# acmater/prograph

Hardware: AMD Instinct MI355X
Metric: sequence-pairs/s (higher is better)
Workload: dtype u8; 1 GPU; cfg3: N=200000 L=64 Hamming, kNN k=16; N=200000, L=64, rows_per_gpu=200000, alphabet=5-bit tokens 1..20, parallelism=rowblock1, engine=mfma

## Files before the change

### prograph_amd/csrc/pg_api.hip

```cpp
#include "pg_common.h"
#include "pg_mm.h"
#include "pg_plan.h"
#include "../../include/prograph_hip.h"

#include <dlfcn.h>
#include <math.h>
#include <rccl/rccl.h>
#include <stdio.h>
#include <stdlib.h>
#include <string.h>
#include <atomic>
#include <mutex>

static thread_local char g_err[256] = "";

void pg_set_error(const char *msg) { snprintf(g_err, sizeof(g_err), "%s", msg); }

extern char **environ;
static PgKnobs read_knobs() { return pg_knobs_read(environ); }

#define PG_MAX_DEVICES 64
static int cu_count() {
  static std::atomic<int> cus[PG_MAX_DEVICES];
  int dev = 0;
  if (hipGetDevice(&dev) != hipSuccess) return 0;
  const bool cached = dev >= 0 && dev < PG_MAX_DEVICES;
  if (cached && cus[dev].load(std::memory_order_relaxed) > 0) return cus[dev].load(std::memory_order_relaxed);
  hipDeviceProp_t prop;
  if (hipGetDeviceProperties(&prop, dev) != hipSuccess) return 0;
  if (cached) cus[dev].store(prop.multiProcessorCount, std::memory_order_relaxed);
  return prop.multiProcessorCount;
}

extern "C" {

int pg_version(void) { return PG_ABI_VERSION; }
const char *pg_last_error(void) { return g_err; }

int pg_device_info(int *cus, int *wave, char *arch, int arch_len) {
  int dev = 0;
  hipDeviceProp_t prop;
  hipError_t e = hipGetDevice(&dev);
  if (e != hipSuccess) return pg_launched((int)e, "hipGetDevice");
  e = hipGetDeviceProperties(&prop, dev);
  if (e != hipSuccess) return pg_launched((int)e, "hipGetDeviceProperties");
  if (cus) *cus = prop.multiProcessorCount;
  if (wave) *wave = prop.warpSize;
  if (arch && arch_len > 0) snprintf(arch, (size_t)arch_len, "%s", prop.gcnArchName);
  return 0;
}

int64_t pg_npad(int64_t n) { return n <= 0 ? 256 : ((n + 255) / 256) * 256; }
int pg_ngroups(int l) { return plan_ngroups(l); }
int pg_nchunks(int l, int bits) { return plan_nchunks(l, bits); }
int64_t pg_planes_bytes(int64_t n, int l, int bits) { return ((int64_t)pg_nchunks(l, bits) * 16 + PG_AUX_BYTES) * pg_npad(n); }
int64_t pg_workspace_bytes(int64_t nrows) { return workspace_bytes(nrows, cu_count(), read_knobs()); }

}

struct SymPlanArgs {
  long long nb, nst, slots;
  int piece, pmin;
  int4 *plan;
  u32 *pieceStart;
  uint4 *zero;
  long long zero4;
  unsigned grid;
};
static __device__ __forceinline__ void sym_plan_workgroup(unsigned vb, unsigned vgrid, const SymPlanArgs &a) {
  __shared__ u32 waveTotal[16];
  const int t = threadIdx.x, lane = t & 63, wv = t >> 6;
  if (vb > 0) {
    for (long long i = (long long)(vb - 1) * 1024 + t; i < a.zero4; i += (long long)(vgrid - 1) * 1024) a.zero[i] = make_uint4(0u, 0u, 0u, 0u);
    return;
  }
  const long long nb = a.nb, per = (nb + 1023) / 1024, b0 = t * per, b1 = b0 + per < nb ? b0 + per : nb;
  const bool few = per <= 4;
  u32 np4 = 0u, mine = 0;
  if (few) {
#pragma unroll 1
    for (int j = 0; b0 + j < b1; ++j) {
      const u32 np = (u32)sym_block_pieces(b0 + j, a.nst, a.slots, a.piece, a.pmin);
      np4 |= np << (8 * j);
      mine += np;
    }
  } else {
#pragma clang loop vectorize(disable) interleave(disable) unroll(disable)
    for (long long b = b0; b < b1; ++b) mine += (u32)sym_block_pieces(b, a.nst, a.slots, a.piece, a.pmin);
  }
  u32 incl = mine;
#pragma unroll
  for (int o = 1; o < 64; o <<= 1) {
    const u32 x = (u32)__shfl_up((int)incl, o);
    incl += lane >= o ? x : 0u;
  }
  if (lane == 63) waveTotal[wv] = incl;
  __syncthreads();
  u32 front = 0, total = 0;
#pragma unroll
  for (int i = 0; i < 16; ++i) {
    const u32 x = waveTotal[i];
    front += i < wv ? x : 0u;
    total += x;
  }
  u32 at = front + incl - mine;
  auto entries = [&](long long b, int np) {
    a.pieceStart[b] = at;
#pragma unroll 1
    for (int q = 0; q < np; ++q, ++at) {
      int f, e;
      sym_piece_range(b, a.nst, np, q, &f, &e);
      a.plan[at] = make_int4((int)b, f, e, q);
    }
  };
  if (few) {
#pragma unroll 1
    for (int j = 0; b0 + j < b1; ++j) entries(b0 + j, (int)((np4 >> (8 * j)) & 0xFFu));
  } else {
#pragma clang loop vectorize(disable) interleave(disable) unroll(disable)
    for (long long b = b0; b < b1; ++b) entries(b, sym_block_pieces(b, a.nst, a.slots, a.piece, a.pmin));
  }
  if (t == 1023) a.pieceStart[nb] = total;
}
__global__ __launch_bounds__(1024) void pg_knn_sym_plan_kernel(SymPlanArgs a) { sym_plan_workgroup(blockIdx.x, gridDim.x, a); }
extern "C" {
int64_t pg_knn_sym_plan(int64_t n, int64_t slots, int piece, int piece_min, int32_t *out, int64_t max_passes) {
  if (n <= 0 || slots <= 0) return pg_fail(PG_E_BADARG, "pg_knn_sym_plan: bad argument");
  return sym_plan_host(n, slots, piece, piece_min > 0 ? piece_min : (int)read_knobs().symPieceMin.v, out, max_passes);
}
int64_t pg_knn_sym_plan_device(int64_t n, int64_t slots, int piece, int piece_min, int32_t *plan_out, uint32_t *piece_start_out,
                               int64_t max_passes, void *stream) {
  if (n <= 0 || n > PG_MAX_N_KNN || slots <= 0 || !plan_out || !piece_start_out) return pg_fail(PG_E_BADARG, "pg_knn_sym_plan_device: bad argument");
  const int pmin = piece_min > 0 ? piece_min : (int)read_knobs().symPieceMin.v;
  const int64_t passes = sym_plan_host(n, slots, piece, pmin, nullptr, 0);
  if (passes > max_passes) return pg_fail(PG_E_BADARG, "pg_knn_sym_plan_device: the plan has more passes than max_passes");
  SymPlanArgs a = {(n + 63) / 64, (n + PG_MM_ST - 1) / PG_MM_ST, slots, piece, pmin, (int4 *)plan_out, piece_start_out, nullptr, 0, 1u};
  pg_knn_sym_plan_kernel<<<dim3(1), dim3(1024), 0, (hipStream_t)stream>>>(a);
  if (int rc = pg_launched("pg_knn_sym_plan_kernel")) return rc;
  return passes;
}
}

#define PG_PACK_SEQS 64
#define PG_PACK_LD 68

__host__ __device__ __forceinline__ unsigned long long pg_transpose8(unsigned long long x) {
  unsigned long long t;
  t = (x ^ (x >> 7)) & 0x00AA00AA00AA00AAull;  x = x ^ t ^ (t << 7);
  t = (x ^ (x >> 14)) & 0x0000CCCC0000CCCCull; x = x ^ t ^ (t << 14);
  t = (x ^ (x >> 28)) & 0x00000000F0F0F0F0ull; x = x ^ t ^ (t << 28);
  return x;
}

template <typename T, int B>
__global__ __launch_bounds__(256) void pg_pack_kernel(const T *__restrict__ src, long long n, int l, long long ld,
                                                      const long long *__restrict__ rows, u32 *__restrict__ planes,
                                                      long long npad, int ng, int nq, u32 *flags,
                                                      const unsigned char *__restrict__ lut = nullptr,
                                                      unsigned char *__restrict__ tokOut = nullptr) {
  constexpr int E = (int)sizeof(T), PER = 16 / E;
  __shared__ __attribute__((aligned(16))) u32 words[PG_PACK_SEQS * PG_PACK_LD];
  const long long s0 = (long long)blockIdx.x * PG_PACK_SEQS;
  const int tid = threadIdx.x;
  const bool vec = !lut && ((unsigned long long)src & 15ull) == 0 && ((ld * E) & 15ll) == 0;
  for (int item = tid; item < PG_PACK_SEQS * ng; item += 256) {
    const int sl = item / ng, g = item - sl * ng;
    const long long s = s0 + sl;
    unsigned long long x[4] = {0, 0, 0, 0}, high = 0;
    if (s < n) {
      const T *row = src + (rows ? rows[s] : s) * ld;
      if (vec && g * 32 + 32 <= l) {
        const uint4 *r16 = reinterpret_cast<const uint4 *>(row + g * 32);
#pragma unroll
        for (int c = 0; c < 32 / PER; ++c) {
          const uint4 v = r16[c];
          T e[PER];
          __builtin_memcpy(e, &v, 16);
#pragma unroll
          for (int i = 0; i < PER; ++i) {
            const int j = c * PER + i;
            const unsigned long long t = (unsigned long long)(long long)e[i];
            high |= t;
            x[j >> 3] |= (t & 0xFFull) << (8 * (j & 7));
          }
        }
      } else {
#pragma unroll
        for (int j = 0; j < 32; ++j) {
          const int pos = g * 32 + j;
          if (pos < l) {
            long long v = (long long)row[pos];
            if (lut) {
              v = lut[(unsigned char)v];
              if (tokOut) tokOut[s * (long long)l + pos] = (unsigned char)v;
            }
            high |= (unsigned long long)v;
            x[j >> 3] |= ((unsigned long long)v & 0xFFull) << (8 * (j & 7));
          }
        }
      }
    }
    if (high >> B) atomicOr(flags, 1u);
#pragma unroll
    for (int i = 0; i < 4; ++i) x[i] = pg_transpose8(x[i]);
#pragma unroll
    for (int p = 0; p < B; ++p) {
      const u32 w = (u32)((x[0] >> (8 * p)) & 0xFFull) | (u32)((x[1] >> (8 * p)) & 0xFFull) << 8 |
                    (u32)((x[2] >> (8 * p)) & 0xFFull) << 16 | (u32)((x[3] >> (8 * p)) & 0xFFull) << 24;
      words[sl * PG_PACK_LD + p * ng + g] = w;
    }
  }
  __syncthreads();
  const int nw = ng * B;
  for (int item = tid; item < PG_PACK_SEQS * nq; item += 256) {
    const int q = item / PG_PACK_SEQS, sl = item % PG_PACK_SEQS;
    uint4 v = *reinterpret_cast<const uint4 *>(&words[sl * PG_PACK_LD + 4 * q]);
    if (4 * q + 1 >= nw) v.y = 0;
    if (4 * q + 2 >= nw) v.z = 0;
    if (4 * q + 3 >= nw) v.w = 0;
    reinterpret_cast<uint4 *>(planes)[(long long)q * npad + s0 + sl] = v;
  }
  const int sl = tid & 63;
  const long long s = s0 + sl;
  if (tid < 64) {
    u32 sigw[2] = {0, 0};
    for (int g = 0; g < ng; ++g) sigw[g & 1] ^= words[sl * PG_PACK_LD + g];
    const unsigned long long sig = pg_sig54(sigw[0], sigw[1]);
    const u32 lo = (u32)sig, hi = (u32)(sig >> 32) | (s < n ? 0xFFC00000u : 0u);
    uint4 *e = reinterpret_cast<uint4 *>(planes + (long long)nq * npad * 4) + (s >> 5) * 64 + (s & 31);
    e[0] = make_uint4(pg_nib8(lo) << 1, pg_nib8(lo >> 8) << 1, pg_nib8(lo >> 16) << 1, pg_nib8(lo >> 24) << 1);
    e[32] = make_uint4(pg_nib8(hi) << 1, pg_nib8(hi >> 8) << 1, pg_nib8(hi >> 16) << 1, pg_nib8(hi >> 24) << 1);
  } else if (tid < 128) {
    u32 fold[8] = {0, 0, 0, 0, 0, 0, 0, 0};
#pragma unroll
    for (int p = 0; p < B; ++p)
      for (int g = 0; g < ng; ++g) fold[p] ^= words[sl * PG_PACK_LD + p * ng + g];
    uint4 *f = reinterpret_cast<uint4 *>(planes + (long long)nq * npad * 4) + npad * 2;
    f[s] = make_uint4(fold[0], fold[1], fold[2], fold[3]);
    f[npad + s] = make_uint4(fold[4], fold[5], fold[6], fold[7]);
  }
}

#define PG_SCAN_TILE 2048

template <typename T>
__device__ __forceinline__ long long scan_val(const T *in, long long i, long long n) {
  return i < n ? (long long)(in[i] != 0 ? (sizeof(T) == 1 ? 1 : in[i]) : 0) : 0;
}

__device__ __forceinline__ long long wave_incl_scan(long long v, int lane) {
#pragma unroll
  for (int o = 1; o < 64; o <<= 1) {
    long long t = __shfl_up(v, o);
    if (lane >= o) v += t;
  }
  return v;
}

__device__ __forceinline__ long long block_excl_scan(long long v, long long &total) {
  __shared__ long long wsum[4];
  const int lane = threadIdx.x & 63, wv = threadIdx.x >> 6;
  const long long inc = wave_incl_scan(v, lane);
  if (lane == 63) wsum[wv] = inc;
  __syncthreads();
  long long base = 0;
  for (int w = 0; w < wv; ++w) base += wsum[w];
  total = wsum[0] + wsum[1] + wsum[2] + wsum[3];
  __syncthreads();
  return base + inc - v;
}

template <typename T>
__global__ __launch_bounds__(256) void pg_scan_partials(const T *__restrict__ in, long long n, long long *partials) {
  const long long b0 = (long long)blockIdx.x * PG_SCAN_TILE;
  long long s = 0;
#pragma unroll
  for (int j = 0; j < 8; ++j) s += scan_val(in, b0 + threadIdx.x * 8 + j, n);
  long long total;
  block_excl_scan(s, total);
  if (threadIdx.x == 0) partials[blockIdx.x] = total;
}

__global__ __launch_bounds__(256) void pg_scan_single(long long *partials, long long nb) {
  long long carry = 0;
  for (long long c0 = 0; c0 < nb; c0 += 256) {
    const long long i = c0 + threadIdx.x;
    const long long v = i < nb ? partials[i] : 0;
    long long total;
    const long long ex = block_excl_scan(v, total);
    if (i < nb) partials[i] = carry + ex;
    carry += total;
  }
  if (threadIdx.x == 0) partials[nb] = carry;
}

template <typename T, int MODE>
__global__ __launch_bounds__(256) void pg_scan_apply(const T *__restrict__ in, long long n, const long long *partials,
                                                     long long nb, long long *out, long long *count) {
  const long long b0 = (long long)blockIdx.x * PG_SCAN_TILE;
  long long v[8], s = 0;
#pragma unroll
  for (int j = 0; j < 8; ++j) { v[j] = scan_val(in, b0 + threadIdx.x * 8 + j, n); s += v[j]; }
  long long total;
  long long ex = block_excl_scan(s, total) + partials[blockIdx.x];
#pragma unroll
  for (int j = 0; j < 8; ++j) {
    const long long i = b0 + threadIdx.x * 8 + j;
    if (i < n) {
      if (MODE == 0) out[i] = ex;
      else if (v[j]) out[ex] = i;
    }
    ex += v[j];
  }
  if (blockIdx.x == 0 && threadIdx.x == 0) {
    if (MODE == 0) out[n] = partials[nb];
    if (count) *count = partials[nb];
  }
}

template <int B>
__global__ __launch_bounds__(256) void pg_index_kernel(const u32 *__restrict__ planes, long long n, long long npad, int ng,
                                                       long long ref, const u32 *__restrict__ want, int posMode,
                                                       const u32 *__restrict__ posMask, const u32 *__restrict__ notMask,
                                                       unsigned char *distOut, u64 *hist, unsigned char *flags) {
  __shared__ u32 lh[256];
  lh[threadIdx.x] = 0;
  __syncthreads();
  const long long s = (long long)blockIdx.x * 256 + threadIdx.x;
  if (s < n) {
    u32 d = 0, anyP = 0, anyNot = 0;
    bool allP = true;
    for (int g = 0; g < ng; ++g) {
      u32 t = 0;
#pragma unroll
      for (int p = 0; p < B; ++p) {
        const int w = p * ng + g;
        const long long base = (long long)(w >> 2) * npad;
        t |= planes[(base + s) * 4 + (w & 3)] ^ planes[(base + ref) * 4 + (w & 3)];
      }
      d += __builtin_popcount(t);
      if (posMode) {
        const u32 pm = posMask[g], nm = notMask[g];
        anyP |= t & pm;
        allP = allP && ((t & pm) == pm);
        anyNot |= t & nm;
      }
    }
    if (distOut) distOut[s] = (unsigned char)d;
    if (hist) atomicAdd(&lh[d & 255u], 1u);
    if (flags) {
      bool ok = want ? ((want[(d >> 5) & 7u] >> (d & 31u)) & 1u) != 0 : true;
      if (posMode == 1) ok = ok && (anyP != 0) && (anyNot == 0);
      if (posMode == 2) ok = ok && allP && (anyNot == 0);
      flags[s] = ok ? 1 : 0;
    }
  }
  __syncthreads();
  if (hist && lh[threadIdx.x]) atomicAdd((unsigned long long *)&hist[threadIdx.x], (unsigned long long)lh[threadIdx.x]);
}

__device__ __forceinline__ double wave_sum(double v) {
#pragma unroll
  for (int o = 32; o > 0; o >>= 1) v += __shfl_down(v, o);
  return v;
}

__global__ __launch_bounds__(256) void pg_csr_row_stats_kernel(const long long *__restrict__ indptr,
                                                               const int *__restrict__ indices,
                                                               const unsigned char *__restrict__ w8,
                                                               const float *__restrict__ wf, long long nrows,
                                                               long long row0, const double *__restrict__ f, double *deg,
                                                               double *sf, double *swf, double *selfw, double *colsum) {
  const int lane = threadIdx.x & 63;
  const long long row = (long long)blockIdx.x * 4 + (threadIdx.x >> 6);
  if (row >= nrows) return;
  const long long a = indptr[row], b = indptr[row + 1];
  double d = 0, s1 = 0, s2 = 0, sw = 0;
  for (long long e = a + lane; e < b; e += 64) {
    const double w = w8 ? (double)w8[e] : (wf ? (double)wf[e] : 1.0);
    const int col = indices[e];
    if (col < 0) continue;
    const double fj = f ? f[col] : 0.0;
    d += w; s1 += fj; s2 += w * fj;
    if (col == row0 + row) sw += w;
    if (colsum) atomicAdd(&colsum[col], w);
  }
  d = wave_sum(d); s1 = wave_sum(s1); s2 = wave_sum(s2); sw = wave_sum(sw);
  if (lane == 0) {
    if (deg) deg[row] = d;
    if (sf) sf[row] = s1;
    if (swf) swf[row] = s2;
    if (selfw) selfw[row] = sw;
  }
}

static int check_l(int l, int bits = 8, bool exact = false) {
  if (l <= 0) return pg_fail(PG_E_BADARG, "sequence length must be positive");
  const int maxg = bits == 5 ? PG_MAX_L_5BIT / 32 + 1 : PG_MAX_L / 32;
  if ((l + 31) / 32 > maxg || (exact && l > (bits == 5 ? PG_MAX_L_5BIT : PG_MAX_L)))
    return pg_fail(PG_E_TOOLONG, "sequence length exceeds the native limit (128 tokens, 255 with 5 bit planes)");
  return 0;
}
static int check_bits(int b) {
  if (b != PG_BITS_5 && b != PG_BITS_8) return pg_fail(PG_E_BADARG, "bits must be 5 or 8");
  return 0;
}

static void eps_interval(int cmp, double eps, u32 *lo, u32 *span, long long dmin = 1) {
  const long long INF = 1000000;
  long long l = dmin, h = INF;
  switch (cmp) {
    case PG_CMP_LE: h = (long long)floor(eps); break;
    case PG_CMP_LT: h = (long long)ceil(eps) - 1; break;
    case PG_CMP_EQ:
      if (floor(eps) == eps) { l = (long long)eps; h = (long long)eps; } else { l = 1; h = 0; }
      break;
    case PG_CMP_GE: l = (long long)ceil(eps); break;
    case PG_CMP_GT: l = (long long)floor(eps) + 1; break;
  }
  if (l < dmin) l = dmin;
  if (h > INF) h = INF;
  if (h < l) { *lo = 0xFFFFFF00u; *span = 0; return; }
  *lo = (u32)l;
  *span = (u32)(h - l);
}

__global__ __launch_bounds__(1024) void pg_decide_kernel(const u32 *counts, int nsample, int wavesPerRow, u32 need, long long ncols,
                                                          int force, u32 *gate, u32 *line, int lineWords, SymPlanArgs ride) {
  if (blockIdx.x > 0) { sym_plan_workgroup(blockIdx.x - 1u, gridDim.x - 1u, ride); return; }
  __shared__ u32 sClustered[16];
  __shared__ unsigned long long sEps[16], sNear[16];
  const int tid = threadIdx.x, s = tid >> 4, sub = tid & 15;
  if (tid < lineWords) line[tid] = 0u;
  u32 nearS = 0, epsS = 0;
  if (s < nsample)
    for (int w = sub; w < wavesPerRow; w += 16) {
      nearS += counts[2 * (s * wavesPerRow + w)];
      epsS += counts[2 * (s * wavesPerRow + w) + 1];
    }
  for (int o = 8; o > 0; o >>= 1) {
// ... 1131 lines not shown
```

### prograph_amd/csrc/pg_plan.h

```cpp
#pragma once
#include "../../include/prograph_hip.h"

#include <math.h>
#include <stdint.h>
#include <stdlib.h>
#include <string.h>
#include <mutex>

#ifdef __HIPCC__
#define PG_HD __host__ __device__
#else
#define PG_HD
#endif

#ifndef PG_MODE_KNN_SHORT
enum { PG_MODE_EPS = 0, PG_MODE_KNN = 1, PG_MODE_EPS_SYM = 2 };
#define PG_MODE_KNN_SHORT 3
#define PG_MODE_KNN_SHORT2 4
#define PG_WG_WAVES 4
#define PG_RB 32
#define PG_RB_KNN 28
#define PG_MM_KL 20
#define PG_MM_RB 32
#define PG_MM_ST 128
#define PG_MM_DENSE_L1 56
#define PG_MM_DENSE_L2 48
#define PG_MM_DIRECT_RUN 8
#define PG_SYM_MAX_PIECES 16
#define PG_SYM_MAX_CAPL 256
#endif
static_assert(PG_MODE_KNN == 1 && PG_MODE_KNN_SHORT == 3 && PG_MODE_KNN_SHORT2 == 4 && PG_WG_WAVES == 4 && PG_RB == 32 &&
                  PG_RB_KNN == 28 && PG_MM_KL == 20 && PG_MM_RB == 32 && PG_MM_ST == 128 && PG_MM_DENSE_L1 == 56 &&
                  PG_MM_DENSE_L2 == 48 && PG_MM_DIRECT_RUN == 8 && PG_SYM_MAX_PIECES == 16 && PG_SYM_MAX_CAPL == 256,
              "pg_plan.h: the host-only copies of the engine's constants follow pg_common.h and pg_mm.h");

PG_HD static inline int sym_dist_bits(uint32_t cap) {
  int b = 0;
  for (uint32_t v = cap > 0 ? cap - 1u : 0u; v; v >>= 1) ++b;
  return b;
}
PG_HD static inline int sym_row_bits(uint32_t cap) { return 28 - sym_dist_bits(cap) < 24 ? 28 - sym_dist_bits(cap) : 24; }
PG_HD static inline bool sym_rows_fit(int64_t n, uint32_t cap) {
  const int rb = sym_row_bits(cap);
  return rb >= 1 && n <= ((int64_t)1 << rb);
}
PG_HD static inline uint32_t sym_entry(uint32_t place, uint32_t d, uint32_t row, int rowBits) { return place << 28 | d << rowBits | row; }
PG_HD static inline uint32_t sym_entry_place(uint32_t e) { return e >> 28; }
PG_HD static inline uint32_t sym_entry_key(uint32_t e, int rowBits) {
  return ((e & 0x0FFFFFFFu) >> rowBits) << 24 | (e & ((1u << rowBits) - 1u));
}
PG_HD static inline uint32_t sym_group_cap(uint32_t n, uint32_t first, uint32_t capL) {
  const uint32_t rows = n > first ? n - first : 0u;
  return (rows < 16u ? rows : 16u) * capL;
}
#define PG_SYM_NONE 0xFFFFFFFFu
template <int W> PG_HD static inline void sym_window_pop(uint32_t (&d)[16], int &used, bool win) {
  static_assert(W == 1 || W == 2 || W == 4 || W == 16, "window widths that divide sixteen");
#ifdef __HIPCC__
#pragma unroll
#endif
  for (int j = 0; j < W - 1; ++j) d[j] = win ? d[j + 1] : d[j];
  d[W - 1] = win ? PG_SYM_NONE : d[W - 1];
  used += win ? 1 : 0;
}
template <int W> PG_HD static inline bool sym_window_empty(int used) { return W < 16 && used == W; }
template <int W> PG_HD static inline void sym_window_refill(uint32_t (&d)[16], int &used) {
  const bool full = sym_window_empty<W>(used);
#ifdef __HIPCC__
#pragma unroll
#endif
  for (int j = 0; j < 16; ++j) d[j] = full ? (j + W < 16 ? d[j + W < 16 ? j + W : 15] : PG_SYM_NONE) : d[j];
  used = full ? 0 : used;
}

#define PG_PROBE_ROWS 64
#define PG_PROBE_WAVES 128
#define PG_PROBE_MIN_N 65536

static inline int plan_ngroups(int l) { return l <= 0 ? 1 : (l + 31) / 32; }
static inline int plan_nchunks(int l, int bits) { return (plan_ngroups(l) * bits + 3) / 4; }

struct PgKnob {
  bool set;
  long long v;
};
struct PgKnobs {
  PgKnob lbFilter, wavesPerCu, rowsPerWave, debugPlan, engine, engineMinRows, probe, probeS, probeW, gateForce, epsOrdered;
  PgKnob knnGuess, mmShort, mmR, mmSplit, mmEvict, mmPieces, mmPiecesAhead, mmPlan, mmTail, mmPersistent, mmL1, mmL2, mmRun;
  PgKnob knnSym, symCapL, symPiece, symPieceMin, symOcc, symDeliver, symEvictLimit, symMergeWgs, symMergeWindow;
};
enum { PG_ENGINE_AUTO = 0, PG_ENGINE_MFMA = 1, PG_ENGINE_VALU = 2 };
enum PgKnobRule { PG_KNOB_ANY, PG_KNOB_CLAMP, PG_KNOB_RANGE, PG_KNOB_WIDE, PG_KNOB_NAME };
struct PgKnobSpec {
  const char *name;
  PgKnob PgKnobs::*field;
  long long dflt, lo, hi;
  PgKnobRule rule;
  const char *what;
};
#define PG_KNOB_MAX 0x7fffffffll
static const PgKnobSpec kPgKnobs[] = {
    {"PG_LB_FILTER", &PgKnobs::lbFilter, 1, 0, 0, PG_KNOB_ANY, "stage-1 lower-bound filter: 1 adaptive, 0 off, 2 forced on"},
    {"PG_WAVES_PER_CU", &PgKnobs::wavesPerCu, 32, 4, 128, PG_KNOB_CLAMP, "VALU engine: size the row split for this many waves per CU (multiples of 4) instead of the cost rule"},
    {"PG_ROWS_PER_WAVE", &PgKnobs::rowsPerWave, 0, 1, PG_KNOB_MAX, PG_KNOB_RANGE, "uniform passes of that many rows (tuning sweeps); present: no column pieces, eps sym by plan_rows"},
    {"PG_DEBUG_PLAN", &PgKnobs::debugPlan, 0, 0, 0, PG_KNOB_ANY, "present: the [pg plan ...] lines on stderr"},
    {"PG_ENGINE", &PgKnobs::engine, PG_ENGINE_AUTO, 0, 0, PG_KNOB_NAME, "mfma / valu forces an engine; present: no probe"},
    {"PG_ENGINE_MIN_ROWS", &PgKnobs::engineMinRows, 0, 0, 0, PG_KNOB_WIDE, "rows from which the MFMA engine runs (default by kind of launch: use_mm_engine); present: no probe"},
    {"PG_PROBE", &PgKnobs::probe, 1, 0, 0, PG_KNOB_ANY, "0: no data probe, the size rules alone"},
    {"PG_PROBE_S", &PgKnobs::probeS, 0, 1, PG_PROBE_ROWS, PG_KNOB_RANGE, "sample rows of the probe (experiments)"},
    {"PG_PROBE_W", &PgKnobs::probeW, 0, 1, PG_PROBE_WAVES, PG_KNOB_RANGE, "waves per sample row of the probe (experiments)"},
    {"PG_GATE_FORCE", &PgKnobs::gateForce, -1, 0, 0, PG_KNOB_ANY, "the probe's decision is forced (tests): bit 0 gate[0], bit 1 gate[1]"},
    {"PG_EPS_ORDERED", &PgKnobs::epsOrdered, 0, 0, 0, PG_KNOB_ANY, "not 0: eps slots in column order (NsqParams::epsOrdered)"},
    {"PG_KNN_GUESS", &PgKnobs::knnGuess, 0, 0, 0, PG_KNOB_ANY, "the optimistic stage-1 cap (default by engine and length); present: no probe"},
    {"PG_MM_SHORT", &PgKnobs::mmShort, 1, 0, 0, PG_KNOB_ANY, "0: keep the 64-lane lists, no short-list instance (A/B runs)"},
    {"PG_MM_R", &PgKnobs::mmR, 0, 0, 0, PG_KNOB_ANY, "1 / 2 forces 32-row / 64-row passes; present: no gated 32-row alternative"},
    {"PG_MM_SPLIT", &PgKnobs::mmSplit, 1, 0, 0, PG_KNOB_ANY, "0: no column pieces, all rows in plain passes"},
    {"PG_MM_EVICT", &PgKnobs::mmEvict, 1, 0, 0, PG_KNOB_ANY, "0: rows that lose their cap finish inside the pass (no eviction, hence no pieces and no symmetric sweep)"},
    {"PG_MM_PIECES", &PgKnobs::mmPieces, 0, 2, 16, PG_KNOB_RANGE, "column pieces per row block (experiments; at most 8 beyond 64 row blocks)"},
    {"PG_MM_PIECES_AHEAD", &PgKnobs::mmPiecesAhead, 1, 0, 0, PG_KNOB_ANY, "0: the pieces always go through the pass counter"},
    {"PG_MM_PLAN", &PgKnobs::mmPlan, 0, 0, 0, PG_KNOB_ANY, "A/B of the pass rule: 2 = round 2's spreading rule everywhere, 1 = the waves-per-SIMD rule for eps too"},
    {"PG_MM_TAIL", &PgKnobs::mmTail, 0, 0, 0, PG_KNOB_ANY, "1: round 2's rule also shrinks the passes of the last round"},
    {"PG_MM_PERSISTENT", &PgKnobs::mmPersistent, 1, 0, 0, PG_KNOB_ANY, "0: one wave per pass instead of persistent waves"},
    {"PG_MM_L1", &PgKnobs::mmL1, PG_MM_DENSE_L1, 0, 0, PG_KNOB_ANY, "NsqParams::mmDenseL1"},
    {"PG_MM_L2", &PgKnobs::mmL2, PG_MM_DENSE_L2, 0, 0, PG_KNOB_ANY, "NsqParams::mmDenseL2"},
    {"PG_MM_RUN", &PgKnobs::mmRun, PG_MM_DIRECT_RUN, 1, PG_KNOB_MAX, PG_KNOB_CLAMP, "NsqParams::mmDirectRun"},
    {"PG_KNN_SYM", &PgKnobs::knnSym, -1, 0, 0, PG_KNOB_ANY, "symmetric kNN sweep: 0 off, 1 forced wherever the MFMA engine runs the short-list kNN"},
    {"PG_KNN_SYM_CAPL", &PgKnobs::symCapL, PG_SYM_MAX_CAPL, 8, PG_SYM_MAX_CAPL, PG_KNOB_CLAMP, "symmetric sweep: delivered keys per row"},
    {"PG_KNN_SYM_PIECE", &PgKnobs::symPiece, 0, 0, 0, PG_KNOB_ANY, "symmetric sweep: fixed piece length in super-tiles (default: guided)"},
    {"PG_KNN_SYM_PIECE_MIN", &PgKnobs::symPieceMin, 32, 4, PG_KNOB_MAX, PG_KNOB_CLAMP, "symmetric sweep: the guided rule's shortest piece"},
    {"PG_KNN_SYM_OCC", &PgKnobs::symOcc, 0, 1, 4, PG_KNOB_RANGE, "symmetric sweep: waves per SIMD the plan counts on"},
    {"PG_KNN_SYM_DELIVER", &PgKnobs::symDeliver, 1, 0, 0, PG_KNOB_ANY, "0: timing experiments, wrong results"},
    {"PG_KNN_SYM_EVICT_LIMIT", &PgKnobs::symEvictLimit, 0, 0, 0, PG_KNOB_WIDE, "evicted rows up to which the sweep's results stand (default: a sixteenth of the rows)"},
    {"PG_KNN_SYM_MERGE_WGS", &PgKnobs::symMergeWgs, 0, 1, PG_KNOB_MAX, PG_KNOB_RANGE, "workgroups of the sweep's merge at most (tests; default and bound: eight a CU)"},
    {"PG_KNN_SYM_MERGE_WINDOW", &PgKnobs::symMergeWindow, 0, 1, 2, PG_KNOB_RANGE, "delivered keys in the window of the merge's rounds: 1 or 2 (tests: the refill runs often; default: four)"},
};

static inline PgKnob pg_knob_parse(const PgKnobSpec &s, const char *text) {
  PgKnob k = {true, s.dflt};
  if (s.rule == PG_KNOB_NAME) {
    k.v = !strcmp(text, "mfma") ? PG_ENGINE_MFMA : (!strcmp(text, "valu") ? PG_ENGINE_VALU : PG_ENGINE_AUTO);
    return k;
  }
  const long long x = s.rule == PG_KNOB_WIDE ? atoll(text) : (long long)atoi(text);
  if (s.rule == PG_KNOB_CLAMP) k.v = x < s.lo ? s.lo : (x > s.hi ? s.hi : x);
  else if (s.rule == PG_KNOB_RANGE) k.v = x >= s.lo && x <= s.hi ? x : s.dflt;
  else k.v = x;
  return k;
}
static inline PgKnobs pg_knobs_read(const char *const *env) {
  PgKnobs kn;
  for (const PgKnobSpec &s : kPgKnobs) kn.*(s.field) = PgKnob{false, s.dflt};
  for (; env && *env; ++env) {
    const char *e = *env;
    if (e[0] != 'P' || e[1] != 'G' || e[2] != '_') continue;
    const char *eq = strchr(e, '=');
    if (!eq) continue;
    for (const PgKnobSpec &s : kPgKnobs)
      if (strlen(s.name) == (size_t)(eq - e) && !strncmp(s.name, e, (size_t)(eq - e))) {
        if (!(kn.*(s.field)).set) kn.*(s.field) = pg_knob_parse(s, eq + 1);
        break;
      }
  }
  return kn;
}

#define PG_WS_FLAGS 64
#define PG_WS_GATES 576
#define PG_WS_COUNTS 640
#define PG_WS_PARTIAL (PG_WS_COUNTS + 8 * 64 * 128)
#define PG_SPLIT_MAX_ROWS 8192
#define PG_SPLIT_MIN_ROWS 65536
#define PG_SYM_MIN_N 65536
#define PG_WS_PARTIAL_BYTES ((int64_t)PG_SPLIT_MAX_ROWS * 8 * PG_MM_KL * 4)
static_assert(PG_WS_COUNTS + 8 * PG_PROBE_ROWS * PG_PROBE_WAVES <= PG_WS_PARTIAL, "pg_workspace_bytes");
static inline int64_t ws_evict_offset(int64_t nrows) { return PG_WS_PARTIAL + (nrows > PG_SPLIT_MIN_ROWS ? PG_WS_PARTIAL_BYTES : 0); }
static inline int64_t ws_sym_offset(int64_t nrows) { return (ws_evict_offset(nrows) + 4 * (nrows > 0 ? nrows : 0) + 64 + 255) / 256 * 256; }

PG_HD static inline int sym_block_pieces(long long b, long long nst, long long slots, int piece, int pmin) {
  const long long len = nst - (b >> 1);
  const long long rem = len * (len + 1) - ((b & 1) ? len : 0);
  long long P = piece > 0 ? piece : (rem / (slots > 0 ? slots : 1)) & ~1ll;
  if (piece <= 0 && P < pmin) P = pmin;
  if (P < 3) P = 3;
  if (P > len) P = len > 3 ? len : 3;
  unsigned np = ((unsigned)len + (unsigned)P - 1u) / (unsigned)P;
  if (np > (unsigned)len / 3u) np = (unsigned)len / 3u;
  if (np > PG_SYM_MAX_PIECES) np = PG_SYM_MAX_PIECES;
  return np < 1 ? 1 : (int)np;
}
PG_HD static inline void sym_piece_range(long long b, long long nst, int np, int q, int *first, int *end) {
  const unsigned s0 = (unsigned)(b >> 1), len = (unsigned)nst - s0, unp = (unsigned)np, uq = (unsigned)q;
  *first = q == 0 ? (int)s0 : (int)(2u * ((s0 + len * uq / unp + 1u) / 2u));
  *end = q + 1 == np ? (int)nst : (int)(2u * ((s0 + len * (uq + 1u) / unp + 1u) / 2u));
}
static inline long long sym_plan_host(long long n, long long slots, int piece, int pmin, int32_t *out, long long cap) {
  const long long nb = (n + 63) / 64, nst = (n + PG_MM_ST - 1) / PG_MM_ST;
  struct Memo { long long n, slots, count; int piece, pmin; };
  static std::mutex memoLock;
  static Memo memo[4] = {};
  static int memoNext = 0;
  if (!out) {
    std::lock_guard<std::mutex> g(memoLock);
    for (const Memo &m : memo)
      if (m.n == n && m.slots == slots && m.piece == piece && m.pmin == pmin && m.count > 0) return m.count;
  }
  long long at = 0;
  for (long long b = 0; b < nb; ++b) {
    const int np = sym_block_pieces(b, nst, slots, piece, pmin);
    for (int q = 0; q < np; ++q, ++at) {
      if (!out || at >= cap) continue;
      int f, e;
      sym_piece_range(b, nst, np, q, &f, &e);
      out[4 * at] = (int)b; out[4 * at + 1] = f; out[4 * at + 2] = e; out[4 * at + 3] = q;
    }
  }
  if (!out) {
    std::lock_guard<std::mutex> g(memoLock);
    memo[memoNext] = Memo{n, slots, at, piece, pmin};
    memoNext = (memoNext + 1) % 4;
  }
  return at;
}
static inline long long sym_slots(int occ, int cus, const PgKnobs &kn) {
  if (kn.symOcc.v >= 1) occ = (int)kn.symOcc.v;
  return (long long)(cus > 0 ? cus : 256) * 4 * (occ < 1 ? 1 : (occ > 4 ? 4 : occ));
}
struct SymWs { int64_t plan, pieceStart, lowCount, partial, lowKeys, bytes; long long maxPasses; };
static inline SymWs sym_ws(int64_t n, int cus, const PgKnobs &kn) {
  SymWs w = {0, 0, 0, 0, 0, 0, 0};
  const int env = (int)kn.knnSym.v;
  if (n <= 0 || n > PG_MAX_N_KNN || env == 0 || (env != 1 && n < PG_SYM_MIN_N)) return w;
  auto up = [](int64_t x) { return (x + 255) / 256 * 256; };
  const long long nb = (n + 63) / 64;
  w.maxPasses = sym_plan_host(n, sym_slots(4, cus, kn), (int)kn.symPiece.v, (int)kn.symPieceMin.v, nullptr, 0);
  w.plan = 0;
  w.pieceStart = up(w.plan + 16 * w.maxPasses);
  w.lowCount = up(w.pieceStart + 4 * (nb + 1));
  w.partial = up(w.lowCount + 4 * n);
  w.lowKeys = up(w.partial + w.maxPasses * 64 * PG_MM_KL * 4);
  w.bytes = up(w.lowKeys + n * (int64_t)kn.symCapL.v * 4);
  return w;
}
static inline int64_t workspace_bytes(int64_t nrows, int cus, const PgKnobs &kn) { return ws_sym_offset(nrows) + sym_ws(nrows, cus, kn).bytes; }

struct PassPlan {
  int rowsPerWave, rowsPerPass;
  long long tailFrom;
  int tailRows;
  long long passes;
  long long gridWaves;
  int grid;
  int occ;
};

static inline int waves_per_cu(const PgKnobs &kn) { return (int)(kn.wavesPerCu.v / 4) * 4; }

static inline PassPlan plan_rows(int64_t nrows, int64_t ncols, int cus, int occ, double recBytes, const PgKnobs &kn, int maxRows = PG_RB) {
  long long rpw = 4;
  if (kn.wavesPerCu.set) {
    const long long maxWaves = (long long)cus * waves_per_cu(kn);
    rpw = (nrows + maxWaves - 1) / maxWaves;
    if (rpw < 1) rpw = 1;
    if (rpw >= 4) rpw = (rpw + 3) / 4 * 4;
  } else {
    static const long long kRound[9] = {0, 22, 31, 37, 43, 51, 60, 70, 80};
    if (occ < 1) occ = 1;
    if (occ > 8) occ = 8;
    const double matBytes = recBytes * (double)ncols;
    double bw = 13e12;
    if (matBytes > 0 && matBytes < 48e6) bw *= fmin(4.0, pow(48e6 / matBytes, 0.65));
    double best = -1;
    for (long long r = 4; r <= maxRows; r += 4) {
      const long long nw = (nrows + r - 1) / r;
      const long long wgs = (nw + PG_WG_WAVES - 1) / PG_WG_WAVES;
      const long long n = (wgs + cus - 1) / cus;
      const double valu = 1.21e-11 * (double)(((n / occ) * kRound[occ] + kRound[n % occ]) * (r + 1));
      const double stream = (double)nw * recBytes / bw;
      const double cost = valu > stream ? valu : stream;
      if (best < 0 || cost <= best * 1.0000001) { best = cost; rpw = r; }
    }
  }
  if (kn.rowsPerWave.v > 0) rpw = kn.rowsPerWave.v;
  const long long waves = (nrows + rpw - 1) / rpw;
  const long long passes = (rpw + maxRows - 1) / maxRows;
  PassPlan pl = {};
  pl.occ = occ;
  pl.rowsPerWave = (int)rpw;
  long long rpp = (rpw + passes - 1) / passes;
  if (rpp >= 4) rpp = (rpp + 3) / 4 * 4;
  if (rpp > maxRows) rpp = maxRows;
  pl.rowsPerPass = (int)rpp;
  pl.passes = waves;
  pl.grid = (int)((waves + PG_WG_WAVES - 1) / PG_WG_WAVES);
  pl.gridWaves = (long long)pl.grid * PG_WG_WAVES;
  return pl;
}

static inline bool use_mm_engine(int64_t nrows, const PgKnobs &kn, int l = 64, bool knn = true) {
  if (kn.engine.v == PG_ENGINE_MFMA) return true;
  if (kn.engine.v == PG_ENGINE_VALU) return false;
  const long long dflt = knn ? 20000 : (l <= 32 ? 36000 : 28000);
  const long long thr = kn.engineMinRows.set ? kn.engineMinRows.v : dflt;
  return nrows >= thr;
}

static inline PassPlan plan_mm(int64_t nrows, int cus, const PgKnobs &kn, int rb = PG_MM_RB, int occ = 4, bool knn = false, int uniformRows = 0) {
  long long rpw = rb, tailFrom = (nrows + rb - 1) / rb, tailRows = rb;
  const long long simds = (long long)(cus > 0 ? cus : 256) * 4;
  const long long slots = simds * (occ < 1 ? 1 : occ);
  const int planEnv = (int)kn.mmPlan.v;
  const bool oldPlan = planEnv == 2 || (!knn && planEnv != 1);
  if (kn.rowsPerWave.v > 0 || uniformRows > 0) {
    const int want = kn.rowsPerWave.v > 0 ? (int)kn.rowsPerWave.v : uniformRows;
    rpw = want < rb ? want : rb;
    tailFrom = (nrows + rpw - 1) / rpw; tailRows = rpw;
  } else if (!oldPlan) {
    if (tailFrom <= slots) {
      const long long w = (tailFrom + simds - 1) / simds;
      long long r = (nrows + w * simds - 1) / (w * simds);
      r = (r + 1) / 2 * 2;
      if (r < 4) r = 4;
      if (r > rb) r = rb;
      rpw = r; tailFrom = (nrows + r - 1) / r; tailRows = r;
    }
  } else {
    const long long full = nrows / (slots * rb) * slots;
    const long long rest = nrows - full * rb;
    if (rest > 0 && (full == 0 || kn.mmTail.v == 1)) {
      long long r = (long long)((double)rest / (0.97 * (double)slots)) + 1;
      r = (r + 1) / 2 * 2;
      if (r < 4) r = 4;
      if (r > rb) r = rb;
      if (full == 0 && r < 16) r = 16;
      tailFrom = full; tailRows = r;
    }
  }
  PassPlan pl = {};
  pl.occ = occ;
  pl.rowsPerWave = (int)rpw; pl.rowsPerPass = rb;
  pl.tailFrom = tailFrom; pl.tailRows = (int)tailRows;
  const long long headRows = tailFrom * rpw < nrows ? tailFrom * rpw : nrows;
  const long long waves = tailFrom + (nrows - headRows + tailRows - 1) / tailRows;
  long long gridWaves = waves < slots ? waves : slots;
  if (kn.mmPersistent.v == 0) gridWaves = waves;
  gridWaves = (gridWaves + PG_WG_WAVES - 1) / PG_WG_WAVES * PG_WG_WAVES;
  pl.passes = waves; pl.gridWaves = gridWaves;
  pl.grid = (int)(gridWaves / PG_WG_WAVES);
  return pl;
}

static inline double knn_plan_cost(long long nrows, long long ncols, int cus, int rb, int occ, bool canSplit, long long *mainRows) {
  static const double S1[4] = {0.43, 0.42, 0.37, 0.12}, H1[4] = {0.148, 0.200, 0.294, 0.477};
  static const double S2[4] = {0.64, 0.69, 0.64, 0.54}, H2[4] = {0.229, 0.292, 0.404, 0.557};
  const bool big = rb > PG_MM_RB;
  const double c = (double)ncols / 1e5, kPieces = 0.04 * c;
  auto T = [&](long long w) { return (big ? S2 : S1)[w - 1] + (big ? H2 : H1)[w - 1] * c; };
  const long long simds = (long long)(cus > 0 ? cus : 256) * 4;
  occ = occ < 1 ? 1 : (occ > 4 ? 4 : occ);
  const long long passes = (nrows + rb - 1) / rb, slots = simds * occ, maxRem = 128ll * rb;
  *mainRows = nrows;
  if (passes <= slots) {
    const long long w = (passes + simds - 1) / simds;
    if (canSplit && w >= 3 && nrows - (w - 1) * simds * rb <= maxRem) {
      *mainRows = (w - 1) * simds * rb;
      return T(w - 1) + kPieces;
    }
    return T(w);
  }
  const long long full = nrows / (slots * rb), rem = nrows - full * slots * rb;
  double t = (double)full * T(occ);
  if (rem > 0) {
    if (canSplit && rem <= maxRem) {
      *mainRows = full * slots * rb;
      t += kPieces;
    } else {
      t += T(((rem + rb - 1) / rb + simds - 1) / simds);
    }
  }
  return t;
}

static inline bool probe_enabled(const PgKnobs &kn) { return kn.probe.v != 0 && !kn.engine.set && !kn.engineMinRows.set; }

struct KnnShape {
  int64_t nrows, ncols, row0;
  bool samePlanes;
  int l, bits, k, first;
  bool floorKeys, lastKeys;
  bool workspace;
};
struct KnnHw {
  int cus;
  int occValu;
  int occMm32;
  int occMm64;
  int occSym;
};
struct KnnPlan {
  bool mm;
  uint32_t guess;
  uint32_t guessValu;
  bool probe;
  PassPlan valu;
  bool shortList, two;
  int mode, rb;
  long long mainRows;
  PassPlan main;
  PassPlan launch;
  uint32_t symGateMask, mainGateMask;
  bool evict;
  int64_t evictOffset;
  int evictGrid;
  uint32_t evictGateMask;
  bool split;
  long long nb;
  int pieces;
  bool piecesAhead;
  unsigned pieceMergeGrid;
  bool sym;
  long long symSlots, symPasses, symNb, symNst, symGridWaves, symLimit, symZero4;
  int symPiece, symPieceMin;
  uint32_t symCapL;
  int symRowBits;
  bool symDeliver;
  unsigned symPlanGrid, symMergeGrid;
  int symMergeWindow;
  bool symPlanRides;
  int64_t symBase;
  SymWs symWs;
  bool alt32;
  PassPlan alt;
};

static inline bool knn_short_list(const KnnShape &s, const PgKnobs &kn) {
  return s.first == 1 && s.k + 1 <= PG_MM_KL && !s.floorKeys && !s.lastKeys && kn.mmShort.v != 0;
}

static inline KnnPlan knn_plan(const KnnShape &s, const KnnHw &hw, const PgKnobs &kn) {
  KnnPlan pl = {};
  const int64_t nrows = s.nrows, ncols = s.ncols;
  const int filter = (int)kn.lbFilter.v, nq = plan_nchunks(s.l, s.bits);
  pl.mm = use_mm_engine(nrows, kn);
  const uint32_t guessMm = s.l > 32 ? 10u : 7u;
  pl.guessValu = 8u;
  pl.guess = kn.knnGuess.set ? (uint32_t)(int)kn.knnGuess.v : (pl.mm ? guessMm : pl.guessValu);
  if (filter == 0) pl.guess = 0;
  if (hw.cus > 0) pl.valu = plan_rows(nrows, ncols, hw.cus, hw.occValu, 16.0 * nq, kn, PG_RB_KNN);
  if (!pl.mm) return pl;
  pl.probe = probe_enabled(kn) && ncols >= PG_PROBE_MIN_N && nrows >= PG_PROBE_MIN_N / 2 && filter != 0 && !kn.knnGuess.set;
  pl.shortList = knn_short_list(s, kn);
  const int occ1 = hw.occMm32, occ2 = pl.shortList ? hw.occMm64 : 0;
  const bool evictOn = kn.mmEvict.v != 0;
  const bool canSplit = pl.shortList && s.workspace && evictOn && pl.guess > 0 && ncols >= 65536 && nrows > PG_SPLIT_MIN_ROWS &&
                        !kn.rowsPerWave.set && kn.mmSplit.v != 0;
  long long main1 = nrows, main2 = nrows;
  const double t1 = knn_plan_cost(nrows, ncols, hw.cus, PG_MM_RB, occ1, canSplit, &main1);
  const double t2 = pl.shortList ? knn_plan_cost(nrows, ncols, hw.cus, 2 * PG_MM_RB, occ2, canSplit, &main2) : 1e30;
  pl.two = pl.shortList && t2 < t1;
  if (kn.mmR.set) pl.two = pl.shortList && kn.mmR.v == 2;
  pl.rb = pl.two ? 2 * PG_MM_RB : PG_MM_RB;
  const int occm = pl.two ? occ2 : occ1;
  pl.mode = pl.two ? PG_MODE_KNN_SHORT2 : (pl.shortList ? PG_MODE_KNN_SHORT : PG_MODE_KNN);
  pl.mainRows = pl.two ? main2 : main1;
  pl.alt32 = pl.two && pl.probe && !kn.mmR.set;
  if (pl.probe) pl.mainGateMask = pl.alt32 ? (1u << 0) : ((1u << 0) | (1u << 2));
  pl.main = plan_mm(pl.mainRows, hw.cus, kn, pl.rb, occm, true);
  pl.launch = pl.main;
  pl.evict = s.first == 1 && !s.floorKeys && !s.lastKeys && pl.guess > 0 && evictOn;
  pl.evictOffset = ws_evict_offset(nrows);
  const long long rowsCap = (long long)(hw.cus > 0 ? hw.cus : 256) * 8;
  pl.evictGrid = (int)(nrows < rowsCap ? nrows : rowsCap);
  pl.symWs = sym_ws(nrows, hw.cus, kn);
  pl.symBase = ws_sym_offset(nrows);
  const bool sym = pl.shortList && pl.evict && s.bits == PG_BITS_5 && nq <= 3 && s.samePlanes && s.row0 == 0 && nrows == ncols &&
                   filter != 0 && pl.symWs.bytes > 0 && (kn.knnSym.v == 1 || pl.two) &&
                   sym_rows_fit(nrows, pl.guess);
  const long long symSlots = sym ? sym_slots(hw.occSym, hw.cus, kn) : 0;
  const long long symPasses = sym ? sym_plan_host(nrows, symSlots, (int)kn.symPiece.v, (int)kn.symPieceMin.v, nullptr, 0) : 0;
  pl.sym = sym && symPasses <= pl.symWs.maxPasses;
  if (pl.sym) {
    pl.symSlots = symSlots; pl.symPasses = symPasses;
    pl.symPiece = (int)kn.symPiece.v; pl.symPieceMin = (int)kn.symPieceMin.v;
    pl.symNb = (nrows + 63) / 64; pl.symNst = (nrows + PG_MM_ST - 1) / PG_MM_ST;
    pl.symGateMask = 1u << 0;
    pl.symCapL = (uint32_t)kn.symCapL.v;
    pl.symRowBits = sym_row_bits(pl.guess);
    pl.symDeliver = kn.symDeliver.v != 0;
    pl.symGridWaves = ((pl.symPasses < pl.symSlots ? pl.symPasses : pl.symSlots) + PG_WG_WAVES - 1) / PG_WG_WAVES * PG_WG_WAVES;
    pl.symZero4 = (nrows + 3) / 4;
    const long long zeroWgs = (pl.symZero4 + 1023) / 1024 < 64 ? (pl.symZero4 + 1023) / 1024 : 64;
    pl.symPlanGrid = (unsigned)(1 + zeroWgs);
    pl.symLimit = kn.symEvictLimit.set ? kn.symEvictLimit.v : nrows / 16;
    const long long mergeWgs = (nrows + 4 * PG_WG_WAVES - 1) / (4 * PG_WG_WAVES);
    long long mergeCap = rowsCap;
    if (kn.symMergeWgs.v >= 1 && kn.symMergeWgs.v < mergeCap) mergeCap = kn.symMergeWgs.v;
    pl.symMergeGrid = (unsigned)(mergeWgs < mergeCap ? mergeWgs : mergeCap);
    pl.symMergeWindow = kn.symMergeWindow.v >= 1 ? (int)kn.symMergeWindow.v : 4;
    pl.symPlanRides = pl.probe;
    if (!pl.probe) pl.mainGateMask = (1u << 0) | (1u << 2);
  }
  pl.evictGateMask = pl.mainGateMask | (pl.sym ? 1u << 3 : 0u);
  pl.split = pl.mainRows < nrows;
  if (pl.split) {
    const long long rem = nrows - pl.mainRows, nb = (rem + pl.rb - 1) / pl.rb;
    const long long simds = (long long)(hw.cus > 0 ? hw.cus : 256) * 4;
    int pieces = (int)(simds / nb);
    pieces = pieces > 16 ? 16 : (pieces < 2 ? 2 : pieces);
    if (kn.mmPieces.v >= 2 && kn.mmPieces.v <= (nb <= 64 ? 16 : 8)) pieces = (int)kn.mmPieces.v;
    pl.nb = nb; pl.pieces = pieces;
    pl.launch.passes = pl.main.passes + nb * pieces;
    pl.launch.tailFrom = pl.launch.passes; pl.launch.tailRows = pl.rb;
    pl.piecesAhead = pl.main.passes + nb * pieces <= simds * occm && kn.mmPiecesAhead.v != 0;
    if (pl.piecesAhead) {
      pl.launch.gridWaves = (pl.launch.passes + PG_WG_WAVES - 1) / PG_WG_WAVES * PG_WG_WAVES;
      pl.launch.grid = (int)(pl.launch.gridWaves / PG_WG_WAVES);
    }
    pl.pieceMergeGrid = (unsigned)((rem + 4 * PG_WG_WAVES - 1) / (4 * PG_WG_WAVES));
  }
  if (pl.alt32) pl.alt = plan_mm(nrows, hw.cus, kn, PG_MM_RB, occ1, true);
  return pl;
}
```

Measured before the change: 41770 billion sequence-pairs/s.

## Split symmetric kNN plan writing across several workgroups

The symmetric plan kernel used to emit every plan entry from a single 1024-thread workgroup. Now 8 workgroups each redundantly compute the full prefix scan of piece counts and then write plan entries only for their own slice of blocks, with a shared-memory table of start offsets. Zeroing workgroups are shifted to start after the planning ones. This shortens the serial planning tail before the main kernel, at the cost of repeating the scan work in every planning workgroup.

```diff
diff --git a/prograph_amd/csrc/pg_api.hip b/prograph_amd/csrc/pg_api.hip
--- a/prograph_amd/csrc/pg_api.hip
+++ b/prograph_amd/csrc/pg_api.hip
@@ -68,14 +68,19 @@
   unsigned grid;
 };
 static __device__ __forceinline__ void sym_plan_workgroup(unsigned vb, unsigned vgrid, const SymPlanArgs &a) {
+  constexpr unsigned P = PG_SYM_PLAN_WGS;
+  constexpr int kShare = 4096 / (int)P + 2;
   __shared__ u32 waveTotal[16];
+  __shared__ u32 shareAt[kShare];
   const int t = threadIdx.x, lane = t & 63, wv = t >> 6;
-  if (vb > 0) {
-    for (long long i = (long long)(vb - 1) * 1024 + t; i < a.zero4; i += (long long)(vgrid - 1) * 1024) a.zero[i] = make_uint4(0u, 0u, 0u, 0u);
+  if (vb >= P) {
+    for (long long i = (long long)(vb - P) * 1024 + t; i < a.zero4; i += (long long)(vgrid - P) * 1024) a.zero[i] = make_uint4(0u, 0u, 0u, 0u);
     return;
   }
   const long long nb = a.nb, per = (nb + 1023) / 1024, b0 = t * per, b1 = b0 + per < nb ? b0 + per : nb;
   const bool few = per <= 4;
+  long long sb0, sb1;
+  sym_plan_share(nb, vb, P, &sb0, &sb1);
   u32 np4 = 0u, mine = 0;
   if (few) {
 #pragma unroll 1
@@ -115,12 +120,28 @@
   };
   if (few) {
 #pragma unroll 1
-    for (int j = 0; b0 + j < b1; ++j) entries(b0 + j, (int)((np4 >> (8 * j)) & 0xFFu));
+    for (int j = 0; b0 + j < b1; ++j) {
+      const long long b = b0 + j;
+      if (b >= sb0 && b <= sb1) shareAt[b - sb0] = at;
+      at += (np4 >> (8 * j)) & 0xFFu;
+    }
+    if (t == 0 && sb1 == nb) shareAt[nb - sb0] = total;
+    __syncthreads();
+#pragma unroll 1
+    for (long long i = t; sb0 + i < sb1; i += 1024) {
+      at = shareAt[i];
+      entries(sb0 + i, (int)(shareAt[i + 1] - at));
+    }
   } else {
+    const long long c0 = b0 > sb0 ? b0 : sb0, c1 = b1 < sb1 ? b1 : sb1;
 #pragma clang loop vectorize(disable) interleave(disable) unroll(disable)
-    for (long long b = b0; b < b1; ++b) entries(b, sym_block_pieces(b, a.nst, a.slots, a.piece, a.pmin));
-  }
-  if (t == 1023) a.pieceStart[nb] = total;
+    for (long long b = b0; c0 < c1 && b < c1; ++b) {
+      const int np = sym_block_pieces(b, a.nst, a.slots, a.piece, a.pmin);
+      if (b >= c0) entries(b, np);
+      else at += (u32)np;
+    }
+  }
+  if (vb == P - 1u && t == 1023) a.pieceStart[nb] = total;
 }
 __global__ __launch_bounds__(1024) void pg_knn_sym_plan_kernel(SymPlanArgs a) { sym_plan_workgroup(blockIdx.x, gridDim.x, a); }
 extern "C" {
@@ -134,8 +155,8 @@
   const int pmin = piece_min > 0 ? piece_min : (int)read_knobs().symPieceMin.v;
   const int64_t passes = sym_plan_host(n, slots, piece, pmin, nullptr, 0);
   if (passes > max_passes) return pg_fail(PG_E_BADARG, "pg_knn_sym_plan_device: the plan has more passes than max_passes");
-  SymPlanArgs a = {(n + 63) / 64, (n + PG_MM_ST - 1) / PG_MM_ST, slots, piece, pmin, (int4 *)plan_out, piece_start_out, nullptr, 0, 1u};
-  pg_knn_sym_plan_kernel<<<dim3(1), dim3(1024), 0, (hipStream_t)stream>>>(a);
+  SymPlanArgs a = {(n + 63) / 64, (n + PG_MM_ST - 1) / PG_MM_ST, slots, piece, pmin, (int4 *)plan_out, piece_start_out, nullptr, 0, PG_SYM_PLAN_WGS};
+  pg_knn_sym_plan_kernel<<<dim3(PG_SYM_PLAN_WGS), dim3(1024), 0, (hipStream_t)stream>>>(a);
   if (int rc = pg_launched("pg_knn_sym_plan_kernel")) return rc;
   return passes;
 }
diff --git a/prograph_amd/csrc/pg_plan.h b/prograph_amd/csrc/pg_plan.h
--- a/prograph_amd/csrc/pg_plan.h
+++ b/prograph_amd/csrc/pg_plan.h
@@ -192,6 +192,14 @@
   const unsigned s0 = (unsigned)(b >> 1), len = (unsigned)nst - s0, unp = (unsigned)np, uq = (unsigned)q;
   *first = q == 0 ? (int)s0 : (int)(2u * ((s0 + len * uq / unp + 1u) / 2u));
   *end = q + 1 == np ? (int)nst : (int)(2u * ((s0 + len * (uq + 1u) / unp + 1u) / 2u));
+}
+#ifndef PG_SYM_PLAN_WGS
+#define PG_SYM_PLAN_WGS 8
+#endif
+static_assert(PG_SYM_PLAN_WGS >= 1 && PG_SYM_PLAN_WGS <= 16, "planning workgroups: the share table is 4096 / P + 2 words");
+PG_HD static inline void sym_plan_share(long long nb, unsigned w, unsigned P, long long *first, long long *end) {
+  *first = nb * (long long)w / (long long)P;
+  *end = nb * (long long)(w + 1u) / (long long)P;
 }
 static inline long long sym_plan_host(long long n, long long slots, int piece, int pmin, int32_t *out, long long cap) {
   const long long nb = (n + 63) / 64, nst = (n + PG_MM_ST - 1) / PG_MM_ST;
@@ -489,7 +497,7 @@
     pl.symGridWaves = ((pl.symPasses < pl.symSlots ? pl.symPasses : pl.symSlots) + PG_WG_WAVES - 1) / PG_WG_WAVES * PG_WG_WAVES;
     pl.symZero4 = (nrows + 3) / 4;
     const long long zeroWgs = (pl.symZero4 + 1023) / 1024 < 64 ? (pl.symZero4 + 1023) / 1024 : 64;
-    pl.symPlanGrid = (unsigned)(1 + zeroWgs);
+    pl.symPlanGrid = (unsigned)(PG_SYM_PLAN_WGS + zeroWgs);
     pl.symLimit = kn.symEvictLimit.set ? kn.symEvictLimit.v : nrows / 16;
     const long long mergeWgs = (nrows + 4 * PG_WG_WAVES - 1) / (4 * PG_WG_WAVES);
     long long mergeCap = rowsCap;
```

Result: no change. 42150 billion sequence-pairs/s (median of 6 runs) (+0.9%).
